# chrischoy/DeepGlobalRegistration

Measured on AMD Instinct MI355X. Metric: pair registrations/sec (FCGF x2 + 1-NN + 6-D inlier net + gate + weighted Procrustes + SE(3) refinement), higher is better.
Workload: dtype f32 results via 2 x f16 split operands (3 f16 MFMA products per MAC, f32 accumulate); k = 1 convs, kNN re-evaluation and registration in exact f32, SVD in f64

## Files before the change

### deepglobalregistration_amd/csrc/conv_os.hip

```cpp
#include <stdlib.h>

#include <type_traits>

#include "dgr_internal.h"
#include "split.h"

typedef float f32x4 __attribute__((ext_vector_type(4)));
typedef int i32x4 __attribute__((ext_vector_type(4)));
typedef unsigned int u32x2 __attribute__((ext_vector_type(2)));
typedef __bf16 bf16x8 __attribute__((ext_vector_type(8)));
typedef _Float16 f16x8 __attribute__((ext_vector_type(8)));
typedef _Float16 f16x2 __attribute__((ext_vector_type(2)));

#ifdef DGR_OS_STAGE_CLK
__device__ unsigned long long dgr_os_stage_clk[8];
#define DGR_OS_CLK(i) do { if (threadIdx.x == 0) { const unsigned long long t_ = __builtin_amdgcn_s_memrealtime(); atomicAdd(&dgr_os_stage_clk[i], t_ - t_prev); t_prev = t_; } } while (0)
extern "C" int dgr_debug_os_stage_clk(unsigned long long *out8, int reset) {
  if (out8 && hipMemcpyFromSymbol(out8, HIP_SYMBOL(dgr_os_stage_clk), 8 * sizeof(unsigned long long)) != hipSuccess) return -1;
  if (reset) { unsigned long long z[8] = {0, 0, 0, 0, 0, 0, 0, 0}; if (hipMemcpyToSymbol(HIP_SYMBOL(dgr_os_stage_clk), z, sizeof(z)) != hipSuccess) return -1; }
  return 0;
}
#else
#define DGR_OS_CLK(i) do { } while (0)
#endif
// ... 225 lines not shown
  for (int q = 0; q < NQ; ++q) {
    const int t = q / PPT, h = q % PPT;
    land(q + 1);
    gather(min(q + 2, NQ - 1));
    if (PPT == 1 || h == 0) {
#pragma unroll
      for (int u = 0; u < GW; ++u) acc[u] = f32x4{0.f, 0.f, 0.f, 0.f};
    }
#pragma unroll
    for (int u = 0; u < GW; ++u) {
      const int n_rows = __builtin_amdgcn_readfirstlane(grp[GP * t + rb0 + u]) >> 16;
      __builtin_amdgcn_sched_barrier(0);
      if (u == 0 || n_rows > 0) mfma_group(u, q & 1);
      wstep(q + 1, u, w[u]);
    }
    if (PPT == 1 || h == PPT - 1) {
#pragma unroll
      for (int u = 0; u < GW; ++u) {
        const int info = grp[GP * t + rb0 + u];
        if ((lane & 15) < (info >> 16)) {
          const int e = ((info >> 8) & 255) + (lane & 15);
          float *p = &acc_s[out_loc[info & 255][e]][16 * cw + 4 * (lane >> 4)];
          f32x4 v = *reinterpret_cast<f32x4 *>(p);
          if constexpr (PM == 2) {
            const float f = __builtin_bit_cast(float, 0x7f000000u - __builtin_bit_cast(uint32_t, in_scale[info & 255][e])) * a.w_unscale;
            v += acc[u] * f;
          } else {
            v += acc[u];
          }
          *reinterpret_cast<f32x4 *>(p) = v;
        }
      }
    }
    __syncthreads();
  }
  DGR_OS_CLK(2);
#ifdef DGR_OS_STAGE_CLK
  if (threadIdx.x == 0) { atomicAdd(&dgr_os_stage_clk[4], 1ull); atomicAdd(&dgr_os_stage_clk[5], (unsigned long long)NQ); }
#endif
  const float out_lo = a.out_relu ? 0.f : -__builtin_inff();
  static_assert(MB * (CS / 4) % THREADS == 0 || THREADS % (CS / 4) == 0, "row lanes stay inside a wave");
  for (int e0 = 0; e0 < MB * (CS / 4); e0 += THREADS) {
    const int e = e0 + tid;
    const bool live = e < MB * (CS / 4);
    const int r = live ? e / (CS / 4) : 0, c = (e % (CS / 4)) * 4;
    uint32_t mx = 0;
    if (live && row0 + r < n_out) {
      f32x4 v = *reinterpret_cast<const f32x4 *>(&acc_s[r][c]);
      v.x = fmaxf(v.x, out_lo); v.y = fmaxf(v.y, out_lo); v.z = fmaxf(v.z, out_lo); v.w = fmaxf(v.w, out_lo);
      *reinterpret_cast<f32x4 *>(a.out + (row0 + r) * a.out_ld + slice * CS + c) = v;
      const i32x4 b = __builtin_bit_cast(i32x4, v);
      mx = max(max((uint32_t)b.x & 0x7fffffffu, (uint32_t)b.y & 0x7fffffffu), max((uint32_t)b.z & 0x7fffffffu, (uint32_t)b.w & 0x7fffffffu));
    }
    if (a.out_amax || a.out_amax2) {
#pragma unroll
      for (int d = CS / 8; d >= 1; d >>= 1) mx = max(mx, (uint32_t)__shfl_xor((int)mx, d, 64));
      if (live && (e % (CS / 4)) == 0 && row0 + r < n_out) {
        if (a.out_amax) atomicMax(a.out_amax + row0 + r, mx);
        if (a.out_amax2) atomicMax(a.out_amax2 + row0 + r, mx);
      }
    }
  }
  DGR_OS_CLK(3);
}

template <int CP, int CS, int MB, int CK, int TM>
static int launch_os(const ConvOsArgs &ka, int64_t n_out_cap, hipStream_t stream) {
  constexpr int GW = (MB >= 64 && CP <= 64) ? 1 : TM / 16;
  int64_t blocks = dgr_ceil_div(n_out_cap, MB);
  blocks = (blocks + 7) / 8 * 8;
  dim3 grid((unsigned)blocks, (unsigned)(ka.cout / CS));
  constexpr int threads = CS * 4 * (TM / 16 / GW);
  if (ka.wb3 && ka.row_amax)
    sparse_conv_os<CP, CS, MB, CK, TM, 2, GW><<<grid, threads, 0, stream>>>(ka);
  else
    sparse_conv_os<CP, CS, MB, CK, TM, 0, GW><<<grid, threads, 0, stream>>>(ka);
  DGR_LAUNCH_CHECK();
  return DGR_OK;
}

int dgr_conv_os_launch(const DgrConvOsLaunch &a, hipStream_t stream, const char **kernel_name) {
  if (a.dense) return dgr_conv_dense_launch(a, stream, kernel_name);
  if (a.up) return dgr_conv_up_launch(a, stream, kernel_name);
  DGR_REQUIRE(a.nbr && a.nbr->built && a.nbr->K == 27, "output-stationary conv: no neighbour table");
  DGR_REQUIRE((a.cin & 3) == 0 && (a.in_ld & 3) == 0 && (a.out_ld & 3) == 0 && (a.res == nullptr || (a.res_ld & 3) == 0),
              "output-stationary conv: channel counts and row strides must be multiples of 4");
  DGR_REQUIRE(a.cout % 32 == 0 && a.cin == a.cin_pad, "output-stationary conv: Cin = %d, Cout = %d must be multiples of 32",
              a.cin, a.cout);
  DGR_REQUIRE(a.n_in_cap > 0 && a.n_in_cap * (int64_t)a.in_ld < (1ll << 32) / 4 * 4,
              "output-stationary conv: input tensor beyond 32-bit element offsets");
  ConvOsArgs ka;
  ka.in = a.in; ka.out = a.out; ka.w16 = a.w16; ka.shift = a.shift; ka.res = a.res;
  ka.wb3 = dgr_exact_f32() ? nullptr : static_cast<const uint4 *>(a.wb3);
  ka.piece_stride = a.piece_stride;
  ka.row_amax = ka.wb3 ? a.row_amax : nullptr;
  ka.w_unscale = a.w_unscale;
  ka.out_amax = a.out_amax; ka.out_amax2 = a.out_amax2;
  DGR_REQUIRE(!ka.wb3 || ka.row_amax, "output-stationary conv: the split weights need the input rows' maxima");
  ka.nbr = a.nbr->nbr; ka.n_out_dev = a.n_out_dev; ka.n_pad = a.nbr->n_pad;
  ka.in_ld = a.in_ld; ka.in_relu = a.in_relu; ka.out_ld = a.out_ld; ka.out_relu = a.out_relu;
  ka.res_ld = a.res_ld; ka.res_relu = a.res_relu;
  ka.cin = a.cin; ka.cout = a.cout; ka.nb16 = a.cout / 16;
#define DGR_OS_TM 32
#define DGR_OS_MBBIG 64
#define DGR_STR2(x) #x
#define DGR_STR(x) DGR_STR2(x)
#define DGR_OS(CPV, CSV, MBV, CKV)                                                                      \
  do {                                                                                                  \
    constexpr int tm = (MBV) < DGR_OS_TM ? ((MBV) < 32 ? 32 : (MBV)) : DGR_OS_TM;                       \
    if (kernel_name) *kernel_name = ka.row_amax ? "sparse_conv_os<" #CPV ", " #CSV ", " DGR_STR(MBV) ", " DGR_STR(CKV) ", f16x2>"  \
                                                 : "sparse_conv_os<" #CPV ", " #CSV ", " DGR_STR(MBV) ", " DGR_STR(CKV) ", f32>"; \
    return launch_os<CPV, CSV, MBV, CKV, tm>(ka, a.n_out_cap, stream);                                  \
  } while (0)
  const int mb = a.rows_per_block;
  const bool narrow = a.cout == 32;
#define DGR_OS_MB(CPV, CKV)                                                 \
  do {                                                                      \
    if (narrow) { DGR_OS(CPV, 32, DGR_OS_MBBIG, CKV); }                     \
    else if (mb == 64) { DGR_OS(CPV, 64, DGR_OS_MBBIG, CKV); }              \
    else if (mb == 32) { DGR_OS(CPV, 64, 32, CKV); }                        \
    else { DGR_OS(CPV, 64, 16, CKV); }                                      \
  } while (0)
  const bool ck128 = a.phase_channels == 128;
  switch (a.cin_pad) {
    case 32: DGR_OS_MB(32, 32);
    case 64: DGR_OS_MB(64, 64);
    case 128: if (ck128) DGR_OS_MB(128, 128); else DGR_OS_MB(128, 64);
    case 256: if (ck128) DGR_OS_MB(256, 128); else DGR_OS_MB(256, 64);
    default: break;
  }
#undef DGR_OS_MB
#undef DGR_OS
  dgr_set_error("output-stationary conv: no instantiation for Cin (padded) %d", a.cin_pad);
  return DGR_EINVAL;
}
```

### deepglobalregistration_amd/csrc/conv_up.hip

```cpp
#include "dgr_internal.h"
#include "split.h"

typedef float f32x4 __attribute__((ext_vector_type(4)));
typedef float f32x2 __attribute__((ext_vector_type(2)));
typedef int i32x4 __attribute__((ext_vector_type(4)));
typedef _Float16 f16x8 __attribute__((ext_vector_type(8)));
typedef _Float16 f16x2 __attribute__((ext_vector_type(2)));
typedef unsigned int u32x4 __attribute__((ext_vector_type(4)));

struct ConvUpArgs {
  const float *in;
  float *out;
  const float *shift;
  const u32x4 *wb;
  int64_t piece_stride;
  const int32_t *nbr;
  int64_t n_pad;
  const int32_t *perm, *cls_count;
  int64_t cls_cap;
  int in_ld, in_relu, out_ld, out_relu;
  int nb16;
  const uint32_t *row_amax;
  uint32_t *out_amax, *out_amax2;
  float w_unscale;
  uint32_t in_bytes;
};

template <int CIN, int RG, int WAVES>
__global__ void __launch_bounds__(64 * WAVES, 2) sparse_conv_up_f16x2(ConvUpArgs a) {
  constexpr int NCB = 4;
  constexpr int NCH = CIN / 64;
  constexpr int S_T = CIN / 32;
  constexpr int THREADS = 64 * WAVES;
  constexpr int MB = WAVES * RG * 16;
  constexpr int NST = 2 * NCB;
  constexpr int WD = NST;
  __shared__ int nbr_s[8][MB];
  __shared__ int rows_s[MB];

  const int tid = threadIdx.x, lane = tid & 63;
  const int wave = __builtin_amdgcn_readfirstlane(tid >> 6);
  const int slice = blockIdx.y;
  int cls = -1, lb = 0, n_cls = 0;
  {
    int b = blockIdx.x;
#pragma unroll
    for (int c = 0; c < 8; ++c) {
      const int n = a.cls_count[c];
      const int nb = (n + MB - 1) / MB;
      if (cls < 0 && b < nb) { cls = c; lb = b; n_cls = n; }
      b -= nb;
    }
  }
  if (cls < 0) return;
  unsigned long long kpack = 0;
  int NL = 0;
  for (int k = 0; k < 27; ++k) {
    const int dx = k % 3 - 1, dy = (k / 3) % 3 - 1, dz = k / 9 - 1;
    if ((dx != 0) == ((cls & 1) != 0) && (dy != 0) == ((cls & 2) != 0) && (dz != 0) == ((cls & 4) != 0)) {
      kpack |= (unsigned long long)k << (5 * NL);
      ++NL;
    }
  }
  auto k_of = [&](int li) { return (int)((kpack >> (5 * li)) & 31ull); };
  const int NIT = NL * NCH;

  for (int i = tid; i < MB; i += THREADS) {
    const int64_t idx = (int64_t)lb * MB + i;
    rows_s[i] = idx < n_cls ? a.perm[(int64_t)cls * a.cls_cap + idx] : -1;
  }
  __syncthreads();
  for (int e = tid; e < NL * MB; e += THREADS) {
    const int li = e / MB, i = e - li * MB;
    const int r = rows_s[i];
    nbr_s[li][i] = r >= 0 ? a.nbr[(int64_t)k_of(li) * a.n_pad + r] : -1;
  }

  u32x4 rh[WD], rm[WD];
  const u32x4 *wph = a.wb + lane, *wpm = a.wb + a.piece_stride + lane;
  auto wreq = [&](int g, int i) {
    const int gc = min(g, NIT * NST - 1);
    const int it = gc / NST, jj = gc - it * NST;
    const int li = it / NCH, ch = it - li * NCH;
    const int64_t frag = ((int64_t)k_of(li) * S_T + 2 * ch + (jj & 1)) * a.nb16 + slice * NCB + (jj >> 1);
    rh[i] = wph[frag * 64];
    rm[i] = wpm[frag * 64];
  };
  const int lr = lane & 15, lq = lane >> 4;
  f32x4 total[RG][NCB];
#pragma unroll
  for (int cb = 0; cb < NCB; ++cb) {
    const f32x4 sh = a.shift ? *reinterpret_cast<const f32x4 *>(a.shift + 64 * slice + 16 * cb + 4 * lq) : f32x4{0.f, 0.f, 0.f, 0.f};
#pragma unroll
    for (int rg = 0; rg < RG; ++rg) total[rg][cb] = sh;
  }
  __syncthreads();

  const __amdgpu_buffer_rsrc_t in_rsrc = __builtin_amdgcn_make_buffer_rsrc(const_cast<float *>(a.in), 0, a.in_bytes, 0x00020000);
  struct RowSet { f32x4 raw[RG][2][2]; uint32_t mx[RG]; int nv[RG]; };
  auto gather = [&](int it, RowSet &g) {
    const int li = it / NCH, ch = it - li * NCH;
#pragma unroll
    for (int rg = 0; rg < RG; ++rg) {
      const int n = nbr_s[li][(wave * RG + rg) * 16 + (lane >> 2)];
      const int ne = max(n, 0);
      const uint32_t off = n >= 0 ? (uint32_t)n * (uint32_t)(a.in_ld * 4) + 256u * ch + 16u * (lane & 3) : a.in_bytes;
      const uint32_t mv = a.row_amax[ne];
#pragma unroll
      for (int s = 0; s < 2; ++s) {
        g.raw[rg][s][0] = __builtin_bit_cast(f32x4, __builtin_amdgcn_raw_buffer_load_b128(in_rsrc, off + 128 * s, 0, 0));
        g.raw[rg][s][1] = __builtin_bit_cast(f32x4, __builtin_amdgcn_raw_buffer_load_b128(in_rsrc, off + 128 * s + 64, 0, 0));
      }
      g.mx[rg] = mv;
      g.nv[rg] = n;
    }
  };
  RowSet gA;
  gather(0, gA);
#pragma unroll
  for (int i = 0; i < WD; ++i) wreq(i, i);
  const int relu_lo = a.in_relu ? 0 : (int)0x80000000;

  f32x4 tmp[RG][NCB];
#pragma unroll 1
  for (int it = 0; it < NIT; ++it) {
    const int ch = it % NCH;
    f16x8 bh[RG][2], bm[RG][2];
    float fold[RG];
    const int from = 4 * (4 * (lane & 15) + (lane >> 4));
#pragma unroll
    for (int rg = 0; rg < RG; ++rg) {
      const float sx = gA.nv[rg] >= 0 ? dgr_row_scale_of(gA.mx[rg]) : 0.f;
      const float fl = sx != 0.f ? dgr_inv_pow2(sx) * a.w_unscale : 0.f;
      fold[rg] = __builtin_bit_cast(float, __builtin_amdgcn_ds_bpermute(16 * (lane & 15), __builtin_bit_cast(int, fl)));
#pragma unroll
      for (int s = 0; s < 2; ++s) {
        i32x4 hw, mw;
#pragma unroll
        for (int h = 0; h < 2; ++h) {
          const i32x4 v = __builtin_bit_cast(i32x4, gA.raw[rg][s][h]);
#pragma unroll
          for (int u = 0; u < 4; u += 2) {
            const f32x2 xs = f32x2{__builtin_bit_cast(float, max(v[u], relu_lo)), __builtin_bit_cast(float, max(v[u + 1], relu_lo))} * sx;
            const f16x2 hh = __builtin_convertvector(xs, f16x2);
            const f16x2 mm = __builtin_convertvector(xs - __builtin_convertvector(hh, f32x2), f16x2);
            hw[2 * h + u / 2] = __builtin_bit_cast(int, hh);
            mw[2 * h + u / 2] = __builtin_bit_cast(int, mm);
          }
        }
#pragma unroll
        for (int d = 0; d < 4; ++d) {
          hw[d] = __builtin_amdgcn_ds_bpermute(from, hw[d]);
          mw[d] = __builtin_amdgcn_ds_bpermute(from, mw[d]);
        }
        bh[rg][s] = __builtin_bit_cast(f16x8, hw);
        bm[rg][s] = __builtin_bit_cast(f16x8, mw);
      }
    }
    __builtin_amdgcn_sched_barrier(0);
    gather(min(it + 1, NIT - 1), gA);
    __builtin_amdgcn_sched_barrier(0);
    if (ch == 0) {
#pragma unroll
      for (int rg = 0; rg < RG; ++rg)
#pragma unroll
        for (int cb = 0; cb < NCB; ++cb) tmp[rg][cb] = f32x4{0.f, 0.f, 0.f, 0.f};
    }
#pragma unroll
    for (int cb = 0; cb < NCB; ++cb) {
#pragma unroll
      for (int s = 0; s < 2; ++s) {
        const int j = cb * 2 + s;
        const f16x8 wh = __builtin_bit_cast(f16x8, rh[j]);
        const f16x8 wm = __builtin_bit_cast(f16x8, rm[j]);
#pragma unroll
        for (int rg = 0; rg < RG; ++rg) tmp[rg][cb] = __builtin_amdgcn_mfma_f32_16x16x32_f16(wm, bh[rg][s], tmp[rg][cb], 0, 0, 0);
#pragma unroll
        for (int rg = 0; rg < RG; ++rg) tmp[rg][cb] = __builtin_amdgcn_mfma_f32_16x16x32_f16(wh, bm[rg][s], tmp[rg][cb], 0, 0, 0);
#pragma unroll
        for (int rg = 0; rg < RG; ++rg) tmp[rg][cb] = __builtin_amdgcn_mfma_f32_16x16x32_f16(wh, bh[rg][s], tmp[rg][cb], 0, 0, 0);
        wreq((it + 1) * NST + j, j);
        __builtin_amdgcn_sched_barrier(0);
      }
    }
    if (ch == NCH - 1) {
#pragma unroll
      for (int rg = 0; rg < RG; ++rg)
#pragma unroll
        for (int cb = 0; cb < NCB; ++cb) total[rg][cb] += tmp[rg][cb] * fold[rg];
    }
  }

  const float out_lo = a.out_relu ? 0.f : -__builtin_inff();
#pragma unroll
  for (int rg = 0; rg < RG; ++rg) {
    const int64_t row = rows_s[(wave * RG + rg) * 16 + lr];
    uint32_t mx = 0;
    if (row >= 0) {
#pragma unroll
      for (int cb = 0; cb < NCB; ++cb) {
        f32x4 v = total[rg][cb];
        v.x = fmaxf(v.x, out_lo); v.y = fmaxf(v.y, out_lo); v.z = fmaxf(v.z, out_lo); v.w = fmaxf(v.w, out_lo);
        *reinterpret_cast<f32x4 *>(a.out + row * a.out_ld + 64 * slice + 16 * cb + 4 * lq) = v;
        const i32x4 b = __builtin_bit_cast(i32x4, v);
        mx = max(mx, max(max((uint32_t)b.x & 0x7fffffffu, (uint32_t)b.y & 0x7fffffffu), max((uint32_t)b.z & 0x7fffffffu, (uint32_t)b.w & 0x7fffffffu)));
      }
    }
    if (a.out_amax || a.out_amax2) {
      mx = max(mx, (uint32_t)__shfl_xor((int)mx, 16, 64));
      mx = max(mx, (uint32_t)__shfl_xor((int)mx, 32, 64));
      if (lq == 0 && row >= 0) {
        if (a.out_amax) atomicMax(a.out_amax + row, mx);
        if (a.out_amax2) atomicMax(a.out_amax2 + row, mx);
      }
    }
  }
}

bool dgr_conv_up_supported(int cin, int cin_pad, int cout) {
  return cin == cin_pad && (cin == 128 || cin == 256) && cout % 64 == 0 && cout >= 64;
}

int dgr_conv_up_launch(const DgrConvOsLaunch &a, hipStream_t stream, const char **kernel_name) {
  DGR_REQUIRE(a.nbr && a.nbr->built && a.nbr->K == 27 && a.nbr->perm && a.nbr->cls_count,
              "parity-class transposed conv: no neighbour table with a class row list");
  DGR_REQUIRE(dgr_conv_up_supported(a.cin, a.cin_pad, a.cout), "parity-class transposed conv: Cin = %d, Cout = %d not built", a.cin, a.cout);
  DGR_REQUIRE(a.wbd && a.row_amax, "parity-class transposed conv: needs the split weights in the dense-tile operand order and the input rows' maxima");
  DGR_REQUIRE(a.res == nullptr, "parity-class transposed conv: no residual input");
  DGR_REQUIRE((a.in_ld & 3) == 0 && (a.out_ld & 3) == 0, "parity-class transposed conv: row strides must be multiples of 4");
  DGR_REQUIRE(a.n_in_cap > 0 && a.n_in_cap * (int64_t)a.in_ld * 4 < (1ll << 31), "parity-class transposed conv: input tensor beyond 2 GB");
  ConvUpArgs ka;
  ka.in = a.in; ka.out = a.out; ka.shift = a.shift;
  ka.wb = static_cast<const u32x4 *>(a.wbd); ka.piece_stride = a.piece_stride;
  ka.nbr = a.nbr->nbr; ka.n_pad = a.nbr->n_pad;
  ka.perm = a.nbr->perm; ka.cls_count = a.nbr->cls_count; ka.cls_cap = a.nbr->cls_cap;
  ka.in_ld = a.in_ld; ka.in_relu = a.in_relu; ka.out_ld = a.out_ld; ka.out_relu = a.out_relu;
  ka.nb16 = a.cout / 16;
  ka.row_amax = a.row_amax; ka.out_amax = a.out_amax; ka.out_amax2 = a.out_amax2;
  ka.w_unscale = a.w_unscale;
  ka.in_bytes = (uint32_t)(a.n_in_cap * (int64_t)a.in_ld * 4);
  constexpr int RG = 2, WAVES = 4, MB = WAVES * RG * 16;
  const dim3 grid((unsigned)(dgr_ceil_div(a.n_out_cap, MB) + 8), (unsigned)(a.cout / 64));
  if (a.cin == 128) {
    if (kernel_name) *kernel_name = "sparse_conv_up_f16x2<128>";
    sparse_conv_up_f16x2<128, RG, WAVES><<<grid, 64 * WAVES, 0, stream>>>(ka);
  } else {
    if (kernel_name) *kernel_name = "sparse_conv_up_f16x2<256>";
    sparse_conv_up_f16x2<256, RG, WAVES><<<grid, 64 * WAVES, 0, stream>>>(ka);
  }
  DGR_LAUNCH_CHECK();
  return DGR_OK;
}
```

### deepglobalregistration_amd/csrc/dgr_internal.h

```cpp
#pragma once
#include <hip/hip_runtime.h>
#include <stdint.h>
#include <stdio.h>
#include <stdlib.h>
#include <string>
#include <vector>

#include "../../include/dgr_hip.h"

void dgr_set_error(const char *fmt, ...);

#define DGR_HIP_CHECK(expr)                                                                  \
  do {                                                                                       \
    hipError_t _e = (expr);                                                                  \
    if (_e != hipSuccess) {                                                                  \
      dgr_set_error("%s:%d: %s failed: %s", __FILE__, __LINE__, #expr, hipGetErrorString(_e)); \
      return DGR_EHIP;                                                                       \
    }                                                                                        \
  } while (0)

#define DGR_CHECK(expr)          \
  do {                           \
    int _r = (expr);             \
    if (_r != DGR_OK) return _r; \
// ... 97 lines not shown
  bool use_nbr = false;
  DgrNbrTable nsame[4];
  DgrNbrTable ndown[3];
  DgrNbrTable nup[3];
  DgrCoordMap cm[4];
  DgrHalfBuckets hb[4];
  DgrKernelMap same[4];
  DgrKernelMap conv1;
  DgrKernelMap down[3];
  int32_t *overflow = nullptr;
};

int dgr_build_maps(DgrArena &arena, const int32_t *coords, int64_t N, int D, int conv1_ks,
                   DgrMapSet *ms, hipStream_t stream, bool skip_conv1_map = false, bool lean = false,
                   bool nbr_tables = false);
int dgr_nbr_counts(const DgrNbrTable &t, const int32_t *n_out_dev, int64_t counts[27]);
int dgr_conv1_probe(DgrArena &arena, const DgrCoordMap &cm, int ks, const float *in, int in_ld, int cin,
                    const float *w_tiled, const float *shift, float *out, int out_ld, int32_t *pair_count,
                    hipStream_t stream, const float *w_compact = nullptr, const char **kernel_name = nullptr,
                    uint32_t *out_amax = nullptr);
int dgr_unique_rows(DgrArena &arena, const int32_t *keys, int64_t n, int nc, int32_t *first_flag,
                    int32_t *rank, int32_t *n_unique_dev, int32_t **table_out, uint32_t *mask_out,
                    hipStream_t stream);
int dgr_exclusive_scan_i32(DgrArena &arena, const int32_t *in, int32_t *out, int64_t n,
                           int32_t *total_out, hipStream_t stream);
constexpr int DGR_SCAN_MAX = 24;
int dgr_exclusive_scan_multi(DgrArena &arena, int count, const int32_t *const *in, int32_t *const *out, const int64_t *n,
                             int32_t *const *total_out, hipStream_t stream);

struct DgrConvLaunch {
  const float *in;
  int in_ld;
  int in_relu;
  float *out;
  int out_ld;
  float *y;
  const float *shift;
  const float *w;
  int cin, cin_pad, cout, cout_pad, K;
  const int32_t *pair_in, *pair_out, *tile_ptr, *rule_ptr;
  const int4 *tile_desc;
  const int32_t *n_rows_dev;
  int64_t tile_bound;
  int l2_normalize = 0;
  unsigned long long *clk = nullptr;
};
int dgr_conv_launch(const DgrConvLaunch &a, int num_cus, hipStream_t stream, const char **kernel_name = nullptr);
struct DgrSplitRows {
  unsigned char *planes = nullptr;
  float *scale = nullptr;
  int channels = 0;
};
bool dgr_conv_wide_supported(int cin_pad, int cin, int cout);
int dgr_conv_wide_launch(const DgrConvLaunch &a, const DgrSplitRows &in, const void *wb, int64_t piece_stride,
                         float w_unscale, int num_cus, hipStream_t stream, const char **kernel_name = nullptr);
int dgr_row_amax(const float *in, int in_ld, int cin, int relu, const int32_t *n_dev, int64_t n_cap, uint32_t *out,
                 hipStream_t stream);
int dgr_split_rows(const float *in, int in_ld, int relu, const int32_t *n_dev, int64_t n_cap, const DgrSplitRows &out,
                   hipStream_t stream);
int dgr_reduce_rows(const float *y, int cout, const int32_t *ptr, const int32_t *pos, const int32_t *n_dev,
                    int64_t n_cap, float *out, int out_ld, const float *shift, const float *res, int res_ld,
                    int res_relu, hipStream_t stream, const DgrSplitRows *split = nullptr, int out_relu = 0);
int dgr_conv_small_cin(const float *in, int in_ld, int in_relu, int cin, const float *w_tiled, const float *w_quad,
                       const float *shift, const DgrKernelMap &km, const int32_t *n_out_dev, int64_t n_out_cap, float *out,
                       int out_ld, hipStream_t stream);
struct DgrConvOsLaunch {
  const float *in; int in_ld, in_relu;
  float *out; int out_ld, out_relu;
  const float *w16, *shift;
  const void *wb3; int64_t piece_stride;
  const void *wbd = nullptr;
  const uint32_t *row_amax = nullptr; float w_unscale = 1.f;
  uint32_t *out_amax = nullptr, *out_amax2 = nullptr;
  int64_t n_in_cap = 0;
  const float *res; int res_ld, res_relu;
  int rows_per_block;
  int phase_channels = 64;
  const DgrNbrTable *nbr;
  const int32_t *n_out_dev;
  int64_t n_out_cap;
  int cin, cin_pad, cout;
  bool dense = false;
  bool up = false;
  const unsigned char *in_dsplit = nullptr;
  unsigned char *out_dsplit = nullptr;
};
int dgr_conv_os_launch(const DgrConvOsLaunch &a, hipStream_t stream, const char **kernel_name = nullptr);
bool dgr_conv_dense_supported(int cin, int cin_pad, int cout);
int dgr_conv_dense_launch(const DgrConvOsLaunch &a, hipStream_t stream, const char **kernel_name = nullptr);
bool dgr_conv_up_supported(int cin, int cin_pad, int cout);
int dgr_conv_up_launch(const DgrConvOsLaunch &a, hipStream_t stream, const char **kernel_name = nullptr);
int dgr_l2_normalize_rows(const float *in, int in_ld, float *out, int out_ld, int c, int relu,
                          const int32_t *n_dev, int64_t n_cap, hipStream_t stream);

struct DgrBatchOutputs {
  const void *ptr[5] = {nullptr, nullptr, nullptr, nullptr, nullptr};
  int64_t numel[5] = {0, 0, 0, 0, 0};
  uint64_t generation = 0;
};

struct DgrEventPool {
  std::vector<hipEvent_t> ev;
  size_t used = 0;
  hipEvent_t next();
  void release();
};

struct dgr_ctx {
  int device = 0;
  int num_cus = 256;
  DgrArena arena;
  bool profiling = false;
  float stage_ms[9] = {0, 0, 0, 0, 0, 0, 0, 0, 0};
  int64_t conv_launches = 0;
  DgrBatchOutputs last;
  std::vector<double> last_T64;
  DgrEventPool events;
  std::vector<std::pair<hipEvent_t, hipEvent_t>> conv_spans, gemm_spans, map3_spans, map6_spans;
  std::vector<float> conv_span_ms, gemm_span_ms;
  std::vector<unsigned long long *> conv_clks;
  std::vector<float> conv_clk_us;
  std::vector<const char *> conv_kinds;
  int32_t *flag_dev = nullptr;
  hipEvent_t wait_ev = nullptr;
  long last_wait_ns = 0;
  double batch_ns_per_row = 0;
  double pairs_ns_per_row = 0;
  unsigned char *pin = nullptr;
  size_t pin_bytes = 0;
  hipStream_t part_stream = nullptr;
  int all_cus = 256;
};

int dgr_ctx_pinned(dgr_ctx *ctx, size_t bytes, unsigned char **out);
int dgr_flag_error(int32_t flag);

int dgr_ctx_wait(dgr_ctx *ctx, hipStream_t stream, long predicted_ns = 0);

int dgr_resunet_forward_impl(dgr_ctx *ctx, dgr_net *net, const int32_t *coords, const float *feats,
                             int64_t N, float *out, hipStream_t stream);
int dgr_ctx_collect_profile(dgr_ctx *ctx);
void dgr_ctx_begin_profile(dgr_ctx *ctx);

int dgr_knn1_batch_impl(dgr_ctx *ctx, const float *F0, const int64_t *off0, const float *F1, const int64_t *off1,
                        int npairs, int C, int squared, int64_t *idx_out, float *dist_out, hipStream_t stream);
int dgr_knn1_impl(dgr_ctx *ctx, const float *F0, int64_t N0, const float *F1, int64_t N1, int C,
                  int squared, int64_t *idx_out, float *dist_out, hipStream_t stream);
int dgr_inlier_inputs_impl(const int32_t *coords0, const float *xyz0, int64_t N0,
                           const int32_t *coords1, const float *xyz1, const int64_t *idx1,
                           int feature_type, int32_t *coords6, float *feats, hipStream_t stream);
int dgr_icp_impl(dgr_ctx *ctx, const float *src, int64_t N0, const float *dst, int64_t N1, double max_dist,
                 const double *T_init, int max_iter, double rel_fitness, double rel_rmse, double *T_out,
                 double *stats_out, hipStream_t stream);
int dgr_ransac_impl(dgr_ctx *ctx, const float *X, const float *Y, int64_t N, double max_dist, int64_t num_hypotheses,
                    uint32_t seed, double *T_out, double *stats_out, hipStream_t stream);
struct DgrIcpJob {
  const float *src = nullptr, *dst = nullptr;
  int64_t N0 = 0, N1 = 0;
  double max_dist = 0;
  int nblocks = 0;
  void *st = nullptr;
  double *P = nullptr, *sorted = nullptr, *partial = nullptr;
  int32_t ncell = 0;
  double host_state[64];
};
int dgr_icp_begin(dgr_ctx *ctx, const float *src, int64_t N0, const float *dst, int64_t N1, double max_dist,
                  const double *T_init_dev , DgrIcpJob *job, hipStream_t stream);
int dgr_icp_run(dgr_ctx *ctx, DgrIcpJob *job, int max_iter, double rel_fitness, double rel_rmse, hipStream_t stream);
void dgr_icp_finish(const DgrIcpJob *job, double *T_out, double *stats_out);
constexpr int DGR_RANSAC_RESULT_DOUBLES = 19;
int dgr_ransac_begin(dgr_ctx *ctx, const float *X, const float *Y, int64_t N, double max_dist, int64_t num_hypotheses,
                     uint32_t seed, double **result_dev, hipStream_t stream);
struct DgrRegResult {
  float R[9];
// ... 15 lines not shown
```

### deepglobalregistration_amd/csrc/net.hip

```cpp
#include <math.h>
#include <stdlib.h>
#include <string.h>

#include <algorithm>
#include <map>
#include <memory>
#include <string>

#include "dgr_internal.h"

static const int CH[5] = {0, 32, 64, 128, 256};
static const int TR[5] = {0, 64, 64, 64, 128};
static constexpr float BN_EPS = 1e-5f;

struct DgrLayer {
  std::string name;
  int K, cin, cout, cin_pad, cout_pad;
  float *w = nullptr;
  float *w16 = nullptr;
  void *w16b = nullptr;
  void *w16d = nullptr;
  int64_t w16b_piece = 0;
  float *wc = nullptr;
  float *wq = nullptr;
// ... 410 lines not shown
  hipStream_t stream;
  DgrMapSet ms;
  bool prof;
  bool l2_next = false;

  float *ybuf = nullptr;

  int conv(int li, const Tensor &in, const DgrKernelMap *km, bool swapped, int lvl_in, int lvl_out,
           const Tensor &out, const Tensor *res) {
    const DgrLayer &L = net->W->layers[li];
    const DgrCoordMap &cin_map = ms.cm[lvl_in], &cout_map = ms.cm[lvl_out];
    DgrConvLaunch a;
    a.in = in.ptr; a.in_ld = in.ld; a.in_relu = in.relu;
    a.out = out.ptr; a.out_ld = out.ld;
    a.y = ybuf; a.shift = L.shift;
    a.w = L.w;
    a.cin = L.cin; a.cin_pad = L.cin_pad; a.cout = L.cout; a.cout_pad = L.cout_pad; a.K = L.K;
    if (km && ms.use_nbr) {
      a.pair_in = a.pair_out = a.tile_ptr = a.rule_ptr = nullptr;
      a.tile_desc = nullptr; a.n_rows_dev = nullptr; a.tile_bound = 0;
    } else if (km) {
      a.pair_in = swapped ? km->pair_out : km->pair_in;
      a.pair_out = swapped ? km->pair_in : km->pair_out;
      a.tile_ptr = km->tile_ptr; a.rule_ptr = km->rule_ptr; a.tile_desc = km->tile_desc;
      a.n_rows_dev = nullptr;
      a.tile_bound = km->pair_cap / DGR_TILE_M + km->K;
      DGR_REQUIRE(km->K == L.K, "layer %s: kernel volume mismatch", L.name.c_str());
      DGR_REQUIRE(!swapped || km->in_ptr, "layer %s: map has no in-major CSR", L.name.c_str());
    } else {
      DGR_REQUIRE(res == nullptr, "identity conv with residual not supported");
      a.pair_in = a.pair_out = a.tile_ptr = a.rule_ptr = nullptr;
      a.tile_desc = nullptr;
      a.n_rows_dev = cout_map.n_dev;
      a.tile_bound = dgr_ceil_div(cout_map.n_cap, DGR_TILE_M);
      a.l2_normalize = l2_next ? 1 : 0;
      l2_next = false;
    }
    hipEvent_t e0 = nullptr, em = nullptr, e1 = nullptr;
    if (prof) {
      e0 = ctx->events.next(); em = ctx->events.next(); e1 = ctx->events.next();
      if (!e0 || !em || !e1) return DGR_EHIP;
      DGR_HIP_CHECK(hipEventRecord(e0, stream));
    }
    if (km && ms.use_nbr) {
      const DgrNbrTable *t = nullptr;
      for (int l = 0; l < 4; ++l)
        if (km == &ms.same[l]) t = &ms.nsame[l];
      for (int l = 0; l < 3; ++l)
        if (km == &ms.down[l]) t = swapped ? &ms.nup[l] : &ms.ndown[l];
      DGR_REQUIRE(t && t->built && L.w16, "layer %s: no neighbour table / 16x16 weights", L.name.c_str());
      DgrConvOsLaunch o;
      o.in = in.ptr; o.in_ld = in.ld; o.in_relu = in.relu;
      o.out = out.ptr; o.out_ld = out.ld; o.out_relu = out.relu;
      o.rows_per_block = lvl_out <= 1 ? 64 : lvl_out == 2 ? (L.cin_pad >= 128 ? 64 : 32) : 16;
      o.phase_channels = (L.cin_pad >= 256 || (L.cin_pad == 128 && lvl_out >= 2)) ? 128 : 64;
      if (const char *e = getenv(lvl_out == 2 ? "DGR_OS_MB2" : lvl_out == 3 ? "DGR_OS_MB3" : "DGR_OS_MB01")) o.rows_per_block = atoi(e);
      if (const char *e = getenv("DGR_OS_CK")) o.phase_channels = atoi(e);
      o.w16 = L.w16; o.shift = L.shift;
      o.wb3 = L.w16b; o.piece_stride = L.w16b_piece;
      o.wbd = L.w16d;
      o.w_unscale = L.w_unscale; o.n_in_cap = cin_map.n_cap;
      if (L.w16b && !dgr_exact_f32()) {
        o.row_amax = in.amax;
        if (!o.row_amax) {
          uint32_t *mx;
          DGR_ALLOC(mx, ctx->arena, uint32_t, cin_map.n_cap);
          DGR_CHECK(dgr_row_amax(in.ptr, in.ld, L.cin, in.relu, cin_map.n_dev, cin_map.n_cap, mx, stream));
          o.row_amax = mx;
        }
      }
      o.out_amax = out.amax; o.out_amax2 = out.amax2;
      o.res = res ? res->ptr : nullptr; o.res_ld = res ? res->ld : 0; o.res_relu = res ? res->relu : 0;
      o.nbr = t; o.n_out_dev = cout_map.n_dev; o.n_out_cap = cout_map.n_cap;
      o.cin = L.cin; o.cin_pad = L.cin_pad; o.cout = L.cout;
      static const bool os_lists = getenv("DGR_OS_LISTS") != nullptr;
      bool same_stride = false;
      for (int l = 0; l < 4; ++l) same_stride = same_stride || t == &ms.nsame[l];
      o.dense = same_stride && o.row_amax && o.wbd && !os_lists && dgr_conv_dense_supported(L.cin, L.cin_pad, L.cout) &&
                cin_map.n_cap * (int64_t)in.ld * 4 < (1ll << 31);
      DGR_REQUIRE(o.dense || (!in.dsplit_only && !out.dsplit_only), "layer %s: dense split rows outside the dense-tile kernel", L.name.c_str());
      static const bool no_up = getenv("DGR_NO_UP") != nullptr;
      o.up = swapped && !o.dense && !no_up && !os_lists && o.row_amax && o.wbd && t->perm && res == nullptr &&
             dgr_conv_up_supported(L.cin, L.cin_pad, L.cout) && cin_map.n_cap * (int64_t)in.ld * 4 < (1ll << 31);
      if (o.dense) {
        o.in_dsplit = in.dsplit;
        o.out_dsplit = out.dsplit;
        if (out.dsplit_only) o.out = nullptr;
      }
      const char *kname = "sparse_conv_os";
      DGR_CHECK(dgr_conv_os_launch(o, stream, &kname));
      if (prof) {
        DGR_HIP_CHECK(hipEventRecord(e1, stream));
        ctx->conv_spans.push_back({e0, e1});
        ctx->gemm_spans.push_back({e0, e1});
        ctx->conv_kinds.push_back(kname);
      }
      LayerRun &r = net->runs[li];
      r = LayerRun();
      r.os = true;
      r.os_launch = o;
      r.nbr = *t;
      r.os_launch.nbr = &r.nbr;
      r.n_in = cin_map.n_dev; r.n_out = cout_map.n_dev; r.K = L.K;
      r.n_out_cap = cout_map.n_cap;
      return DGR_OK;
    }
    const bool small_cin = km && !swapped && !res && L.cin <= 8 && L.cout == 32 && L.cin_pad == 8;
    const char *kname = (L.cin == 6 && L.wq) ? "conv_cin6_quad_kernel" : L.cin == 1 ? "conv_small_cin_row_kernel" : "conv_small_cin_kernel";
    unsigned long long *clk = nullptr;
    const bool wide = L.wb && km;
    if (small_cin)
      DGR_CHECK(dgr_conv_small_cin(in.ptr, in.ld, in.relu, L.cin, L.w, L.wq, L.shift, *km, cout_map.n_dev, cout_map.n_cap,
                                   out.ptr, out.ld, stream));
    else if (wide) {
      DGR_REQUIRE(in.split.planes, "layer %s: the wide-layer kernel needs its input as split rows", L.name.c_str());
      if (prof) {
        DGR_ALLOC(a.clk, ctx->arena, unsigned long long, 2);
        DGR_HIP_CHECK(hipMemsetAsync(a.clk, 0xff, sizeof(unsigned long long), stream));
        DGR_HIP_CHECK(hipMemsetAsync(a.clk + 1, 0, sizeof(unsigned long long), stream));
        clk = a.clk;
      }
      DGR_CHECK(dgr_conv_wide_launch(a, in.split, L.wb, L.wb_piece, L.w_unscale, ctx->num_cus, stream, &kname));
    } else
      DGR_CHECK(dgr_conv_launch(a, ctx->num_cus, stream, &kname));
    if (prof) DGR_HIP_CHECK(hipEventRecord(em, stream));
    DGR_REQUIRE(!out.split.planes || (km && !small_cin), "layer %s: only a reduction can write split rows", L.name.c_str());
    if (km && !small_cin)
      DGR_CHECK(dgr_reduce_rows(ybuf, L.cout, swapped ? km->in_ptr : km->out_ptr, swapped ? km->in_pos : km->out_pos,
                                cout_map.n_dev, cout_map.n_cap, out.split_only ? nullptr : out.ptr, out.ld, L.shift, res ? res->ptr : nullptr,
                                res ? res->ld : 0, res ? res->relu : 0, stream, out.split.planes ? &out.split : nullptr,
                                out.relu));
    if (prof) {
      DGR_HIP_CHECK(hipEventRecord(e1, stream));
      ctx->conv_spans.push_back({e0, e1});
      ctx->gemm_spans.push_back({e0, em});
      ctx->conv_kinds.push_back(kname);
      ctx->conv_clks.resize(ctx->conv_spans.size(), nullptr);
      ctx->conv_clks.back() = clk;
    }
    LayerRun &r = net->runs[li];
    a.clk = nullptr;
    r.launch = a;
    r.split_in = wide ? in.split : DgrSplitRows();
    r.split_out = out.split;
    r.out_relu = out.relu;
    r.split_only = out.split_only;
    r.has_reduce = km != nullptr;
    r.small_cin = small_cin;
    if (km) r.km = *km;
    if (km) {
      r.red_ptr = swapped ? km->in_ptr : km->out_ptr;
      r.red_pos = swapped ? km->in_pos : km->out_pos;
    }
    r.n_out_cap = cout_map.n_cap;
    r.res = res ? res->ptr : nullptr; r.res_ld = res ? res->ld : 0; r.res_relu = res ? res->relu : 0;
    r.rule_ptr = km ? km->rule_ptr : nullptr;
    r.n_in = cin_map.n_dev; r.n_out = cout_map.n_dev; r.K = L.K;
    return DGR_OK;
  }
};

int dgr_resunet_forward_impl(dgr_ctx *ctx, dgr_net *net, const int32_t *coords, const float *feats,
                             int64_t N, float *out, hipStream_t stream) {
  DgrArena &A = ctx->arena;
  Fwd f;
  f.ctx = ctx; f.net = net; f.stream = stream; f.prof = ctx->profiling;
// ... 411 lines not shown
```

Measured before the change: 385.8.

## Route non-dense Cin=128 same-stride convs through all-offsets MFMA kernel

Generalizes the parity-class transposed-conv kernel body into a template with an all-27-offsets mode, adding residual add and an optional 64-bit-address gather path. Same-stride Cin=128 layers that fall back from the dense kernel now use this split-f16 MFMA kernel instead of the generic output-stationary conv. The goal is to reuse the faster pipelined weight-prefetch and gather structure of the up kernel for these layers. It costs larger shared-memory neighbour tables (27 rows) and another kernel variant, and it only applies when the dense path is rejected.

After: 392.0, median of 6. 1.02x the previous value.

```diff
diff --git a/deepglobalregistration_amd/csrc/conv_os.hip b/deepglobalregistration_amd/csrc/conv_os.hip
--- a/deepglobalregistration_amd/csrc/conv_os.hip
+++ b/deepglobalregistration_amd/csrc/conv_os.hip
@@ -331,6 +331,7 @@
 int dgr_conv_os_launch(const DgrConvOsLaunch &a, hipStream_t stream, const char **kernel_name) {
   if (a.dense) return dgr_conv_dense_launch(a, stream, kernel_name);
   if (a.up) return dgr_conv_up_launch(a, stream, kernel_name);
+  if (a.full27) return dgr_conv_full27_launch(a, stream, kernel_name);
   DGR_REQUIRE(a.nbr && a.nbr->built && a.nbr->K == 27, "output-stationary conv: no neighbour table");
   DGR_REQUIRE((a.cin & 3) == 0 && (a.in_ld & 3) == 0 && (a.out_ld & 3) == 0 && (a.res == nullptr || (a.res_ld & 3) == 0),
               "output-stationary conv: channel counts and row strides must be multiples of 4");
diff --git a/deepglobalregistration_amd/csrc/conv_up.hip b/deepglobalregistration_amd/csrc/conv_up.hip
--- a/deepglobalregistration_amd/csrc/conv_up.hip
+++ b/deepglobalregistration_amd/csrc/conv_up.hip
@@ -18,6 +18,10 @@
   int64_t n_pad;
   const int32_t *perm, *cls_count;
   int64_t cls_cap;
+  const int32_t *n_out_dev;
+  int64_t n_out_cap;
+  const float *res;
+  int res_ld, res_relu;
   int in_ld, in_relu, out_ld, out_relu;
   int nb16;
   const uint32_t *row_amax;
@@ -26,8 +30,9 @@
   uint32_t in_bytes;
 };
 
-template <int CIN, int RG, int WAVES>
-__global__ void __launch_bounds__(64 * WAVES, 2) sparse_conv_up_f16x2(ConvUpArgs a) {
+template <int CIN, int RG, int WAVES, bool FULL, bool FAR>
+__device__ __forceinline__ void conv_up_body(const ConvUpArgs &a) {
+  static_assert(FULL || !FAR, "64-bit gather addresses: all-offsets mode only");
   constexpr int NCB = 4;
   constexpr int NCH = CIN / 64;
   constexpr int S_T = CIN / 32;
@@ -35,14 +40,19 @@
   constexpr int MB = WAVES * RG * 16;
   constexpr int NST = 2 * NCB;
   constexpr int WD = NST;
-  __shared__ int nbr_s[8][MB];
+  __shared__ int nbr_s[FULL ? 27 : 8][MB];
   __shared__ int rows_s[MB];
 
   const int tid = threadIdx.x, lane = tid & 63;
   const int wave = __builtin_amdgcn_readfirstlane(tid >> 6);
   const int slice = blockIdx.y;
   int cls = -1, lb = 0, n_cls = 0;
-  {
+  unsigned long long kpack = 0;
+  int NL = 0;
+  if constexpr (FULL) {
+    lb = blockIdx.x; n_cls = (int)min((int64_t)*a.n_out_dev, a.n_out_cap); NL = 27;
+    if ((int64_t)lb * MB >= n_cls) return;
+  } else {
     int b = blockIdx.x;
 #pragma unroll
     for (int c = 0; c < 8; ++c) {
@@ -51,23 +61,21 @@
       if (cls < 0 && b < nb) { cls = c; lb = b; n_cls = n; }
       b -= nb;
     }
-  }
-  if (cls < 0) return;
-  unsigned long long kpack = 0;
-  int NL = 0;
-  for (int k = 0; k < 27; ++k) {
-    const int dx = k % 3 - 1, dy = (k / 3) % 3 - 1, dz = k / 9 - 1;
-    if ((dx != 0) == ((cls & 1) != 0) && (dy != 0) == ((cls & 2) != 0) && (dz != 0) == ((cls & 4) != 0)) {
-      kpack |= (unsigned long long)k << (5 * NL);
-      ++NL;
-    }
-  }
-  auto k_of = [&](int li) { return (int)((kpack >> (5 * li)) & 31ull); };
+    if (cls < 0) return;
+    for (int k = 0; k < 27; ++k) {
+      const int dx = k % 3 - 1, dy = (k / 3) % 3 - 1, dz = k / 9 - 1;
+      if ((dx != 0) == ((cls & 1) != 0) && (dy != 0) == ((cls & 2) != 0) && (dz != 0) == ((cls & 4) != 0)) {
+        kpack |= (unsigned long long)k << (5 * NL);
+        ++NL;
+      }
+    }
+  }
+  auto k_of = [&](int li) { return FULL ? li : (int)((kpack >> (5 * li)) & 31ull); };
   const int NIT = NL * NCH;
 
   for (int i = tid; i < MB; i += THREADS) {
     const int64_t idx = (int64_t)lb * MB + i;
-    rows_s[i] = idx < n_cls ? a.perm[(int64_t)cls * a.cls_cap + idx] : -1;
+    rows_s[i] = idx >= n_cls ? -1 : FULL ? (int)idx : a.perm[(int64_t)cls * a.cls_cap + idx];
   }
   __syncthreads();
   for (int e = tid; e < NL * MB; e += THREADS) {
@@ -94,6 +102,21 @@
 #pragma unroll
     for (int rg = 0; rg < RG; ++rg) total[rg][cb] = sh;
   }
+  if constexpr (FULL) {
+    if (a.res) {
+#pragma unroll
+      for (int rg = 0; rg < RG; ++rg) {
+        const int64_t row = rows_s[(wave * RG + rg) * 16 + lr];
+        if (row < 0) continue;
+#pragma unroll
+        for (int cb = 0; cb < NCB; ++cb) {
+          f32x4 x = *reinterpret_cast<const f32x4 *>(a.res + row * a.res_ld + 64 * slice + 16 * cb + 4 * lq);
+          if (a.res_relu) { x.x = fmaxf(x.x, 0.f); x.y = fmaxf(x.y, 0.f); x.z = fmaxf(x.z, 0.f); x.w = fmaxf(x.w, 0.f); }
+          total[rg][cb] += x;
+        }
+      }
+    }
+  }
   __syncthreads();
 
   const __amdgpu_buffer_rsrc_t in_rsrc = __builtin_amdgcn_make_buffer_rsrc(const_cast<float *>(a.in), 0, a.in_bytes, 0x00020000);
@@ -104,12 +127,21 @@
     for (int rg = 0; rg < RG; ++rg) {
       const int n = nbr_s[li][(wave * RG + rg) * 16 + (lane >> 2)];
       const int ne = max(n, 0);
-      const uint32_t off = n >= 0 ? (uint32_t)n * (uint32_t)(a.in_ld * 4) + 256u * ch + 16u * (lane & 3) : a.in_bytes;
       const uint32_t mv = a.row_amax[ne];
-#pragma unroll
-      for (int s = 0; s < 2; ++s) {
-        g.raw[rg][s][0] = __builtin_bit_cast(f32x4, __builtin_amdgcn_raw_buffer_load_b128(in_rsrc, off + 128 * s, 0, 0));
-        g.raw[rg][s][1] = __builtin_bit_cast(f32x4, __builtin_amdgcn_raw_buffer_load_b128(in_rsrc, off + 128 * s + 64, 0, 0));
+      if constexpr (FAR) {
+        const float *p = a.in + (int64_t)ne * a.in_ld + 64 * ch + 4 * (lane & 3);
+#pragma unroll
+        for (int s = 0; s < 2; ++s) {
+          g.raw[rg][s][0] = *reinterpret_cast<const f32x4 *>(p + 32 * s);
+          g.raw[rg][s][1] = *reinterpret_cast<const f32x4 *>(p + 32 * s + 16);
+        }
+      } else {
+        const uint32_t off = n >= 0 ? (uint32_t)n * (uint32_t)(a.in_ld * 4) + 256u * ch + 16u * (lane & 3) : a.in_bytes;
+#pragma unroll
+        for (int s = 0; s < 2; ++s) {
+          g.raw[rg][s][0] = __builtin_bit_cast(f32x4, __builtin_amdgcn_raw_buffer_load_b128(in_rsrc, off + 128 * s, 0, 0));
+          g.raw[rg][s][1] = __builtin_bit_cast(f32x4, __builtin_amdgcn_raw_buffer_load_b128(in_rsrc, off + 128 * s + 64, 0, 0));
+        }
       }
       g.mx[rg] = mv;
       g.nv[rg] = n;
@@ -138,7 +170,10 @@
         i32x4 hw, mw;
 #pragma unroll
         for (int h = 0; h < 2; ++h) {
-          const i32x4 v = __builtin_bit_cast(i32x4, gA.raw[rg][s][h]);
+          i32x4 v = __builtin_bit_cast(i32x4, gA.raw[rg][s][h]);
+          if constexpr (FAR) {
+            if (gA.nv[rg] < 0) v = i32x4{0, 0, 0, 0};
+          }
 #pragma unroll
           for (int u = 0; u < 4; u += 2) {
             const f32x2 xs = f32x2{__builtin_bit_cast(float, max(v[u], relu_lo)), __builtin_bit_cast(float, max(v[u + 1], relu_lo))} * sx;
@@ -217,8 +252,32 @@
   }
 }
 
+template <int CIN, int RG, int WAVES>
+__global__ void __launch_bounds__(64 * WAVES, 2) sparse_conv_up_f16x2(ConvUpArgs a) {
+  conv_up_body<CIN, RG, WAVES, false, false>(a);
+}
+
+template <int CIN, int RG, int WAVES, bool FAR>
+__global__ void __launch_bounds__(64 * WAVES, 2) sparse_conv_full27_f16x2(ConvUpArgs a) {
+  conv_up_body<CIN, RG, WAVES, true, FAR>(a);
+}
+
 bool dgr_conv_up_supported(int cin, int cin_pad, int cout) {
   return cin == cin_pad && (cin == 128 || cin == 256) && cout % 64 == 0 && cout >= 64;
+}
+
+static void conv_up_args(const DgrConvOsLaunch &a, ConvUpArgs &ka) {
+  ka.in = a.in; ka.out = a.out; ka.shift = a.shift;
+  ka.wb = static_cast<const u32x4 *>(a.wbd); ka.piece_stride = a.piece_stride;
+  ka.nbr = a.nbr->nbr; ka.n_pad = a.nbr->n_pad;
+  ka.perm = a.nbr->perm; ka.cls_count = a.nbr->cls_count; ka.cls_cap = a.nbr->cls_cap;
+  ka.n_out_dev = a.n_out_dev; ka.n_out_cap = a.n_out_cap;
+  ka.res = a.res; ka.res_ld = a.res_ld; ka.res_relu = a.res_relu;
+  ka.in_ld = a.in_ld; ka.in_relu = a.in_relu; ka.out_ld = a.out_ld; ka.out_relu = a.out_relu;
+  ka.nb16 = a.cout / 16;
+  ka.row_amax = a.row_amax; ka.out_amax = a.out_amax; ka.out_amax2 = a.out_amax2;
+  ka.w_unscale = a.w_unscale;
+  ka.in_bytes = (uint32_t)(a.n_in_cap * (int64_t)a.in_ld * 4);
 }
 
 int dgr_conv_up_launch(const DgrConvOsLaunch &a, hipStream_t stream, const char **kernel_name) {
@@ -230,15 +289,7 @@
   DGR_REQUIRE((a.in_ld & 3) == 0 && (a.out_ld & 3) == 0, "parity-class transposed conv: row strides must be multiples of 4");
   DGR_REQUIRE(a.n_in_cap > 0 && a.n_in_cap * (int64_t)a.in_ld * 4 < (1ll << 31), "parity-class transposed conv: input tensor beyond 2 GB");
   ConvUpArgs ka;
-  ka.in = a.in; ka.out = a.out; ka.shift = a.shift;
-  ka.wb = static_cast<const u32x4 *>(a.wbd); ka.piece_stride = a.piece_stride;
-  ka.nbr = a.nbr->nbr; ka.n_pad = a.nbr->n_pad;
-  ka.perm = a.nbr->perm; ka.cls_count = a.nbr->cls_count; ka.cls_cap = a.nbr->cls_cap;
-  ka.in_ld = a.in_ld; ka.in_relu = a.in_relu; ka.out_ld = a.out_ld; ka.out_relu = a.out_relu;
-  ka.nb16 = a.cout / 16;
-  ka.row_amax = a.row_amax; ka.out_amax = a.out_amax; ka.out_amax2 = a.out_amax2;
-  ka.w_unscale = a.w_unscale;
-  ka.in_bytes = (uint32_t)(a.n_in_cap * (int64_t)a.in_ld * 4);
+  conv_up_args(a, ka);
   constexpr int RG = 2, WAVES = 4, MB = WAVES * RG * 16;
   const dim3 grid((unsigned)(dgr_ceil_div(a.n_out_cap, MB) + 8), (unsigned)(a.cout / 64));
   if (a.cin == 128) {
@@ -251,3 +302,34 @@
   DGR_LAUNCH_CHECK();
   return DGR_OK;
 }
+
+bool dgr_conv_full27_supported(int cin, int cin_pad, int cout) {
+  return cin == 128 && dgr_conv_up_supported(cin, cin_pad, cout);
+}
+
+int dgr_conv_full27_launch(const DgrConvOsLaunch &a, hipStream_t stream, const char **kernel_name) {
+  DGR_REQUIRE(a.nbr && a.nbr->built && a.nbr->K == 27 && a.n_out_dev, "all-offsets conv: no neighbour table / row count");
+  DGR_REQUIRE(dgr_conv_full27_supported(a.cin, a.cin_pad, a.cout), "all-offsets conv: Cin = %d, Cout = %d not built", a.cin, a.cout);
+  DGR_REQUIRE(a.wbd && a.row_amax, "all-offsets conv: needs the split weights in the dense-tile operand order and the input rows' maxima");
+  DGR_REQUIRE((a.in_ld & 3) == 0 && (a.out_ld & 3) == 0 && (a.res == nullptr || (a.res_ld & 3) == 0),
+              "all-offsets conv: row strides must be multiples of 4");
+  DGR_REQUIRE(a.n_in_cap > 0, "all-offsets conv: no input row capacity");
+  DGR_REQUIRE(a.n_out_cap <= a.nbr->n_pad, "all-offsets conv: more rows than the neighbour table holds");
+  ConvUpArgs ka;
+  conv_up_args(a, ka);
+  constexpr int RG = 2, WAVES = 4, MB = WAVES * RG * 16;
+  const dim3 grid((unsigned)dgr_ceil_div(a.n_out_cap, MB), (unsigned)(a.cout / 64));
+  static const bool force_far = getenv("DGR_FULL27_FAR") != nullptr;
+  const bool far = force_far || a.n_in_cap * (int64_t)a.in_ld * 4 >= (1ll << 31);
+  if (far) ka.in_bytes = 0;
+#define DGR_FULL27(CINV, FARV, NAME)                                                              \
+  do {                                                                                            \
+    if (kernel_name) *kernel_name = NAME;                                                         \
+    sparse_conv_full27_f16x2<CINV, RG, WAVES, FARV><<<grid, 64 * WAVES, 0, stream>>>(ka);        \
+  } while (0)
+  if (!far) DGR_FULL27(128, false, "sparse_conv_full27_f16x2<128>");
+  else DGR_FULL27(128, true, "sparse_conv_full27_f16x2<128, far>");
+#undef DGR_FULL27
+  DGR_LAUNCH_CHECK();
+  return DGR_OK;
+}
diff --git a/deepglobalregistration_amd/csrc/dgr_internal.h b/deepglobalregistration_amd/csrc/dgr_internal.h
--- a/deepglobalregistration_amd/csrc/dgr_internal.h
+++ b/deepglobalregistration_amd/csrc/dgr_internal.h
@@ -203,6 +203,7 @@
   int cin, cin_pad, cout;
   bool dense = false;
   bool up = false;
+  bool full27 = false;
   const unsigned char *in_dsplit = nullptr;
   unsigned char *out_dsplit = nullptr;
 };
@@ -211,6 +212,8 @@
 int dgr_conv_dense_launch(const DgrConvOsLaunch &a, hipStream_t stream, const char **kernel_name = nullptr);
 bool dgr_conv_up_supported(int cin, int cin_pad, int cout);
 int dgr_conv_up_launch(const DgrConvOsLaunch &a, hipStream_t stream, const char **kernel_name = nullptr);
+bool dgr_conv_full27_supported(int cin, int cin_pad, int cout);
+int dgr_conv_full27_launch(const DgrConvOsLaunch &a, hipStream_t stream, const char **kernel_name = nullptr);
 int dgr_l2_normalize_rows(const float *in, int in_ld, float *out, int out_ld, int c, int relu,
                           const int32_t *n_dev, int64_t n_cap, hipStream_t stream);
 
diff --git a/deepglobalregistration_amd/csrc/net.hip b/deepglobalregistration_amd/csrc/net.hip
--- a/deepglobalregistration_amd/csrc/net.hip
+++ b/deepglobalregistration_amd/csrc/net.hip
@@ -516,6 +516,9 @@
       static const bool no_up = getenv("DGR_NO_UP") != nullptr;
       o.up = swapped && !o.dense && !no_up && !os_lists && o.row_amax && o.wbd && t->perm && res == nullptr &&
              dgr_conv_up_supported(L.cin, L.cin_pad, L.cout) && cin_map.n_cap * (int64_t)in.ld * 4 < (1ll << 31);
+      static const bool no_full27 = getenv("DGR_NO_FULL27") != nullptr;
+      o.full27 = same_stride && !o.dense && !o.up && !no_full27 && !os_lists && o.row_amax && o.wbd &&
+                 dgr_conv_full27_supported(L.cin, L.cin_pad, L.cout);
       if (o.dense) {
         o.in_dsplit = in.dsplit;
         o.out_dsplit = out.dsplit;
```
